# JuliaGenAI/ColBERT.jl

Hardware: AMD Instinct MI355X
Metric: queries/sec, top-1000 on 1M-passage corpus (higher is better)
Workload: dtype f32

## Files before the change

### colbert.jl_amd/csrc/search_kernels.hpp

```cpp
#pragma once
#include <hip/hip_fp16.h>

#include "common.hpp"

namespace clb {

typedef float f32x16 __attribute__((ext_vector_type(16)));
typedef float f32x4 __attribute__((ext_vector_type(4)));

constexpr int kDim = 128;
constexpr int kCentTileStride = 132;
constexpr int kMaxTopK = 16384;

static __global__ __launch_bounds__(128) void centroid_scores_kernel(const float* __restrict__ C,
                                                               const float* __restrict__ Q,
                                                               float* __restrict__ cells, int K, int T,
                                                               int TT, int n_tiles) {
    extern __shared__ __attribute__((aligned(16))) float lds[];
    const int wave = threadIdx.x >> 6, lane = threadIdx.x & 63;
    const int i = lane & 31, h = lane >> 5;
    const int b = blockIdx.y / TT, tt = blockIdx.y % TT;
    const int Tpad = TT * 32;
    float* my = lds + wave * (32 * kCentTileStride);

// ... 358 lines not shown
    uint32_t* bm = bitmap + (size_t)b * W;
    const int w0 = slice * (SB * 1024);
#pragma unroll
    for (int j = 0; j < SB; ++j) {
        const int wi = j * 1024 + tid;
        const uint32_t word = lbm[wi];
        if (w0 + wi < W) bm[w0 + wi] = word;
        int c = __popc(word);
#pragma unroll
        for (int o = 32; o > 0; o >>= 1) c += __shfl_xor(c, o, 64);
        if ((tid & 63) == 0 && c) atomicAdd(&cnt[j], c);
    }
    __syncthreads();
    if (tid < SB && slice * SB + tid < nblk)
        blocksum[(size_t)b * nblk + slice * SB + tid] = cnt[tid];
}

static __global__ __launch_bounds__(kScanBlock) void bitmap_count_kernel(const uint32_t* __restrict__ bitmap,
                                                                  int* __restrict__ blocksum, int W) {
    __shared__ int sh[8];
    const int b = blockIdx.y;
    const uint32_t* bm = bitmap + (size_t)b * W;
    const int w0 = (blockIdx.x * kScanBlock + threadIdx.x) * kWordsPerThread;
    int cnt = 0;
#pragma unroll
    for (int j = 0; j < kWordsPerThread; ++j)
        if (w0 + j < W) cnt += __popc(bm[w0 + j]);
    int total;
    (void)block_exclusive_scan_256(cnt, sh, total);
    if (threadIdx.x == 0) blocksum[(size_t)b * gridDim.x + blockIdx.x] = total;
}

static __global__ __launch_bounds__(kScanBlock) void bitmap_emit_kernel(uint32_t* __restrict__ bitmap,
                                                                 const int* __restrict__ blockcnt,
                                                                 uint32_t* __restrict__ cand,
                                                                 const uint32_t* __restrict__ doc_off,
                                                                 uint2* __restrict__ cand_hdr, int W,
                                                                 size_t cand_cap, int* __restrict__ ncand) {
    __shared__ int sh[8];
    const int b = blockIdx.y;
    int before = 0;
    {
        const int* bc = blockcnt + (size_t)b * gridDim.x;
        const int upto = blockIdx.x == 0 ? (int)gridDim.x : (int)blockIdx.x;
        int part = 0;
        for (int i = threadIdx.x; i < upto; i += kScanBlock) part += bc[i];
        int total_;
        (void)block_exclusive_scan_256(part, sh, total_);
        if (blockIdx.x == 0) { if (threadIdx.x == 0) ncand[b] = total_; }
        else before = total_;
    }
    uint32_t* bm = bitmap + (size_t)b * W;
    const int w0 = (blockIdx.x * kScanBlock + threadIdx.x) * kWordsPerThread;
    uint32_t w[kWordsPerThread];
    int cnt = 0;
#pragma unroll
    for (int j = 0; j < kWordsPerThread; ++j) {
        w[j] = (w0 + j < W) ? bm[w0 + j] : 0u;
        cnt += __popc(w[j]);
    }
    int total;
    int pos = block_exclusive_scan_256(cnt, sh, total) + before;
    uint32_t* out = cand + (size_t)b * cand_cap;
    uint2* hdr = cand_hdr + (size_t)b * cand_cap;
#pragma unroll
    for (int j = 0; j < kWordsPerThread; ++j) {
        uint32_t x = w[j];
        if (x) bm[w0 + j] = 0u;
        while (x) {
            const int bit = __ffs((int)x) - 1;
            x &= x - 1;
            if ((size_t)pos < cand_cap) {
                const uint32_t pid = (uint32_t)((w0 + j) * 32 + bit);
                out[pos] = pid;
                const uint32_t o = doc_off[pid];
                hdr[pos] = make_uint2(o, doc_off[pid + 1] - o);
            }
            ++pos;
        }
    }
}

template <int NBITS>
__device__ __forceinline__ float bucket_weight(uint32_t idx, const float (&w)[4], float wlane) {
    if constexpr (NBITS == 1) {
        return idx ? w[1] : w[0];
    } else if constexpr (NBITS == 2) {
        const float lo = (idx & 1) ? w[1] : w[0];
        const float hi = (idx & 1) ? w[3] : w[2];
        return (idx & 2) ? hi : lo;
    } else {
        return __shfl(wlane, (int)idx, 64);
    }
}

template <int NBITS>
__device__ __forceinline__ void decompress_lane_dims(const float* __restrict__ cent_row ,
                                                     const uint32_t (&R)[NBITS * 4], int g,
                                                     const float (&w)[4], float wlane, float (&x)[32]) {
    float p = 0.f;
#pragma unroll
    for (int s = 0; s < 32; ++s) {
        const int bitpos = 4 * s * NBITS;
        const uint32_t idx = (R[bitpos >> 5] >> ((bitpos & 31) + g * NBITS)) & ((1u << NBITS) - 1u);
        const float v = cent_row[4 * s] + bucket_weight<NBITS>(idx, w, wlane);
        x[s] = v;
        const float sq = v * v;
        p = p + sq;
    }
    const float a = p + __shfl_xor(p, 16, 64);
    const float n2 = a + __shfl_xor(a, 32, 64);
    const float den = sqrtf(n2) + FLT_EPSILON;
#pragma unroll
    for (int s = 0; s < 32; ++s) x[s] = x[s] / den;
}

__device__ __forceinline__ float div_by_reciprocal(float x, float den, float y) {
    const float q0 = x * y;
    const float r = fmaf(-den, q0, x);
    return fmaf(r, y, q0);
}

template <int NBITS>
constexpr int weight_table_floats() { return (1 << NBITS) * 32; }
template <int NBITS>
__device__ __forceinline__ void fill_weight_table(float* tbl, const float* __restrict__ weights) {
    for (int i = threadIdx.x; i < weight_table_floats<NBITS>(); i += blockDim.x) tbl[i] = weights[i >> 5];
}

template <int NBITS>
__device__ __forceinline__ void decompress_lane_dims_fast(const float* __restrict__ cent_row ,
                                                          const uint32_t (&R)[NBITS * 4], int g,
                                                          const float* __restrict__ tbl, float (&x)[32],
                                                          const float* ctile = nullptr, int r = 0) {
    float p = 0.f;
    const float* tbl_lane = tbl + (threadIdx.x & 31);
#pragma unroll
    for (int s = 0; s < 32; ++s) {
        const int bit0 = 4 * s * NBITS;
        const uint32_t idx = __builtin_amdgcn_ubfe(R[bit0 >> 5], (uint32_t)((bit0 & 31) + g * NBITS), (uint32_t)NBITS);
        const float c = ctile ? ctile[(s * 16 + (r ^ (s & 15))) * 4 + ((g + 2 * (((r >> 3) ^ ((s & 15) >> 3)) & 1)) & 3)] : cent_row[4 * s];
        const float val = c + tbl_lane[idx * 32];
        x[s] = val;
        const float sq = val * val;
        p = p + sq;
    }
    const float a = p + __shfl_xor(p, 16, 64);
    const float n2 = a + __shfl_xor(a, 32, 64);
    const float den = sqrtf(n2) + FLT_EPSILON;
    if (__builtin_expect(den > 1e-18f && den < 1e18f, 1)) {
        const float y = 1.0f / den;
#pragma unroll
        for (int s = 0; s < 32; ++s) x[s] = div_by_reciprocal(x[s], den, y);
    } else {
#pragma unroll
        for (int s = 0; s < 32; ++s) x[s] = x[s] / den;
    }
}

constexpr int kMaxMaskedRows = 256;

template <int NBITS>
static __global__ __launch_bounds__(256, 3) void score_exact_kernel(
    const float* __restrict__ C, const float* __restrict__ weights, const uint32_t* __restrict__ codes0,
    const uint8_t* __restrict__ residuals, const uint2* __restrict__ cand_hdr, const float* __restrict__ Q,
    const int* __restrict__ ncand, float* __restrict__ scores, int T, size_t cand_cap,
    const int* __restrict__ list , const int* __restrict__ nlist) {
    constexpr int RD = NBITS * 4;
    __shared__ float tbl[weight_table_floats<NBITS>()];
    __shared__ __attribute__((aligned(16))) float qlds[16 * 64 * 4];
    __shared__ __attribute__((aligned(16))) float ctiles[4 * 512 * 4];
    fill_weight_table<NBITS>(tbl, weights);
    const int b = blockIdx.y;
    const int lane = threadIdx.x & 63;
    const int r = lane & 15, g = lane >> 4;
    const int wave = threadIdx.x >> 6;
    const int wave_global = blockIdx.x * 4 + wave;
    const int nwaves = gridDim.x * 4;
    const int n = list ? nlist[b] : ncand[b];
    const int TT = (T + 31) >> 5;
    const uint2* hdr = cand_hdr + (size_t)b * cand_cap;
    const int* lst = list ? list + (size_t)b * cand_cap : nullptr;
    float* ctile = ctiles + wave * 2048;
    const int c4 = lane & 31, rhalf = lane >> 5;

    auto stage_q = [&](int tt) {
        for (int i = threadIdx.x; i < 16 * 64; i += 256) {
            const int k = i >> 6, l = i & 63;
            const int rr = l & 15, gg = l >> 4;
            const int t0 = tt * 32 + rr, t1 = t0 + 16;
            const float* qa = Q + ((size_t)b * T + (t0 < T ? t0 : T - 1)) * kDim + gg;
            const float* qb = Q + ((size_t)b * T + (t1 < T ? t1 : T - 1)) * kDim + gg;
            float4 v;
            v.x = t0 < T ? qa[8 * k] : 0.f;
            v.y = t1 < T ? qb[8 * k] : 0.f;
            v.z = t0 < T ? qa[8 * k + 4] : 0.f;
            v.w = t1 < T ? qb[8 * k + 4] : 0.f;
            *reinterpret_cast<float4*>(qlds + (size_t)i * 4) = v;
        }
    };
    const float4* qv = reinterpret_cast<const float4*>(qlds) + lane;

#define CLB_REP8(X) X(0) X(1) X(2) X(3) X(4) X(5) X(6) X(7)
#define CLB_ROW_DECL(m) float4 row##m;
#define CLB_ROW_LOAD(m)                                                                                        \
    {                                                                                                          \
        const uint32_t ca = __builtin_amdgcn_readlane(code_rows, 2 * m), cb = __builtin_amdgcn_readlane(code_rows, 2 * m + 1); \
        row##m = *reinterpret_cast<const float4*>(C + (size_t)(rhalf ? cb : ca) * kDim + 4 * c4);              \
    }
#define CLB_ROW_STORE(m)                                                                                       \
    {      \
        float* sl_ = ctile + (c4 * 16 + ((2 * m + rhalf) ^ (c4 & 15))) * 4;                                    \
        const int ro_ = 2 * ((((2 * m + rhalf) >> 3) ^ (c4 >> 3)) & 1);                                        \
        *reinterpret_cast<float2*>(sl_ + ro_) = make_float2(row##m.x, row##m.y);                               \
        *reinterpret_cast<float2*>(sl_ + (ro_ ^ 2)) = make_float2(row##m.z, row##m.w);                         \
    }

    for (int tt = 0; tt < TT; ++tt) {
        __syncthreads();
        stage_q(tt);
        __syncthreads();
        int slot_cur = wave_global < n ? (lst ? lst[wave_global] : wave_global) : 0;
        int slot_nxt = wave_global + nwaves < n ? (lst ? lst[wave_global + nwaves] : wave_global + nwaves) : 0;
        uint2 h_cur = hdr[slot_cur];
        for (int j = wave_global; j < n; j += nwaves) {
            const int slot = slot_cur;
            const uint32_t off = __builtin_amdgcn_readfirstlane(h_cur.x);
            const int len = (int)__builtin_amdgcn_readfirstlane(h_cur.y);
            {
                const int j1 = j + nwaves, j2 = j + 2 * nwaves;
                slot_cur = slot_nxt;
                if (j1 < n) h_cur = hdr[slot_nxt];
                slot_nxt = j2 < n ? (lst ? lst[j2] : j2) : 0;
            }
            float m0 = kNegInf, m1 = kNegInf;
            auto row_at = [&](int el) -> uint32_t { return (uint32_t)(el < len ? el : len - 1); };
            auto code_at = [&](int base) { return codes0[off + row_at(base + r)]; };
            uint32_t Rn[RD];
            auto load_res = [&](int base) {
                const uint32_t e = off + row_at(base + r);
                const uint32_t* rp = reinterpret_cast<const uint32_t*>(residuals + (size_t)e * (RD * 4));
#pragma unroll
                for (int k4 = 0; k4 < RD; k4 += 4) {
                    uint4 v = *reinterpret_cast<const uint4*>(rp + k4);
                    Rn[k4] = v.x; Rn[k4 + 1] = v.y; Rn[k4 + 2] = v.z; Rn[k4 + 3] = v.w;
                }
            };
            uint32_t code_rows = code_at(0);
            uint32_t code_next = code_at(16);
            load_res(0);
            CLB_REP8(CLB_ROW_DECL)
            CLB_REP8(CLB_ROW_LOAD)
            for (int base = 0; base < len; base += 16) {
                uint32_t R[RD];
#pragma unroll
                for (int k4 = 0; k4 < RD; ++k4) R[k4] = Rn[k4];
                CLB_REP8(CLB_ROW_STORE)
                __builtin_amdgcn_wave_barrier();
                if (base + 16 < len) load_res(base + 16);
                float x[32];
                decompress_lane_dims_fast<NBITS>(nullptr, R, g, tbl, x, ctile, r);
                __builtin_amdgcn_wave_barrier();
                code_rows = code_next;
                if (base + 16 < len) { CLB_REP8(CLB_ROW_LOAD) }
                code_next = code_at(base + 32);
                f32x4 a0 = {0.f, 0.f, 0.f, 0.f}, a1 = {0.f, 0.f, 0.f, 0.f};
                float4 qnext = qv[0];
#pragma unroll
                for (int k = 0; k < 16; ++k) {
                    const float4 q = qnext;
                    if (k < 15) qnext = qv[(k + 1) * 64];
                    a0 = __builtin_amdgcn_mfma_f32_16x16x4f32(x[2 * k], q.x, a0, 0, 0, 0);
                    a1 = __builtin_amdgcn_mfma_f32_16x16x4f32(x[2 * k], q.y, a1, 0, 0, 0);
                    a0 = __builtin_amdgcn_mfma_f32_16x16x4f32(x[2 * k + 1], q.z, a0, 0, 0, 0);
                    a1 = __builtin_amdgcn_mfma_f32_16x16x4f32(x[2 * k + 1], q.w, a1, 0, 0, 0);
                }
                m0 = fmaxf(fmaxf(m0, fmaxf(a0[0], a0[1])), fmaxf(a0[2], a0[3]));
                m1 = fmaxf(fmaxf(m1, fmaxf(a1[0], a1[1])), fmaxf(a1[2], a1[3]));
            }
            m0 = fmaxf(m0, __shfl_xor(m0, 16, 64));
            m0 = fmaxf(m0, __shfl_xor(m0, 32, 64));
            m1 = fmaxf(m1, __shfl_xor(m1, 16, 64));
            m1 = fmaxf(m1, __shfl_xor(m1, 32, 64));
            float total = tt == 0 ? 0.f : scores[(size_t)b * cand_cap + slot];
#pragma unroll
            for (int t = 0; t < 32; ++t) {
                const float v = __shfl(t < 16 ? m0 : m1, t & 15, 64);
                if (tt * 32 + t < T) total = total + v;
            }
            if (lane == 0) scores[(size_t)b * cand_cap + slot] = total;
        }
    }
#undef CLB_REP8
#undef CLB_ROW_DECL
#undef CLB_ROW_LOAD
#undef CLB_ROW_STORE
}

struct ExactStepTag {
    int slot;
    int slot1;
    int info;
};
__device__ __forceinline__ uint32_t nth_set_bit_256(unsigned long long w0, unsigned long long w1,
                                                    unsigned long long w2, unsigned long long w3, int n) {
    const int c0 = __popcll(w0), c1 = c0 + __popcll(w1), c2 = c1 + __popcll(w2);
    unsigned long long w = w0;
    int add = 0, loc = n;
    if (n >= c0) { w = w1; add = 64; loc = n - c0; }
    if (n >= c1) { w = w2; add = 128; loc = n - c1; }
    if (n >= c2) { w = w3; add = 192; loc = n - c2; }
    uint32_t x = (uint32_t)w;
    const int cl = __popc(x);
    if (loc >= cl) { x = (uint32_t)(w >> 32); add += 32; loc -= cl; }
#pragma unroll
    for (int width = 16; width >= 1; width >>= 1) {
        const int t = __popc(x & ((1u << width) - 1u));
        if (loc >= t) { x >>= width; add += width; loc -= t; }
    }
    return (uint32_t)add;
}

static __global__ __launch_bounds__(256, 3) void score_exact_flat_kernel(
    const float* __restrict__ C, const float* __restrict__ weights, const uint32_t* __restrict__ codes0,
    const uint8_t* __restrict__ residuals, const uint2* __restrict__ cand_hdr, const float* __restrict__ Q,
    float* __restrict__ scores, int T, size_t cand_cap, const int* __restrict__ list,
    const int* __restrict__ nlist, const unsigned long long* __restrict__ rowmask) {
    constexpr int NBITS = 2;
    __shared__ float tbl[weight_table_floats<NBITS>()];
    __shared__ __attribute__((aligned(16))) float qlds[16 * 64 * 4];
    __shared__ __attribute__((aligned(16))) float ctiles[4 * 512 * 4];
    fill_weight_table<NBITS>(tbl, weights);
    const int lane = threadIdx.x & 63;
    const int r = lane & 15, g = lane >> 4;
    const int wave = __builtin_amdgcn_readfirstlane(threadIdx.x >> 6);
    float* ctile = ctiles + wave * 2048;
    const int c4 = lane & 31, rhalf = lane >> 5;
    const float4* qv = reinterpret_cast<const float4*>(qlds) + lane;

#define CLB_REP8(X) X(0) X(1) X(2) X(3) X(4) X(5) X(6) X(7)
#define CLB_ROW_DECL(m) float4 rowA##m;
#define CLB_ROW_LOAD(P, CODE, m)                                                                               \
    {                                                                                                          \
        const uint32_t ca = __builtin_amdgcn_readlane(CODE, 2 * m), cb = __builtin_amdgcn_readlane(CODE, 2 * m + 1); \
        row##P##m = *reinterpret_cast<const float4*>(C + (size_t)(rhalf ? cb : ca) * kDim + 4 * c4);           \
    }
#define CLB_ROW_LOAD8(P, CODE)                                                                                 \
    CLB_ROW_LOAD(P, CODE, 0) CLB_ROW_LOAD(P, CODE, 1) CLB_ROW_LOAD(P, CODE, 2) CLB_ROW_LOAD(P, CODE, 3)        \
    CLB_ROW_LOAD(P, CODE, 4) CLB_ROW_LOAD(P, CODE, 5) CLB_ROW_LOAD(P, CODE, 6) CLB_ROW_LOAD(P, CODE, 7)
#define CLB_ROW_STORE(P, m)                                                                                    \
    {      \
        float* sl_ = ctile + (c4 * 16 + ((2 * m + rhalf) ^ (c4 & 15))) * 4;                                    \
        const int ro_ = 2 * ((((2 * m + rhalf) >> 3) ^ (c4 >> 3)) & 1);                                        \
        *reinterpret_cast<float2*>(sl_ + ro_) = make_float2(row##P##m.x, row##P##m.y);                         \
        *reinterpret_cast<float2*>(sl_ + (ro_ ^ 2)) = make_float2(row##P##m.z, row##P##m.w);                   \
    }
#define CLB_ROW_STORE8(P)                                                                                      \
    CLB_ROW_STORE(P, 0) CLB_ROW_STORE(P, 1) CLB_ROW_STORE(P, 2) CLB_ROW_STORE(P, 3)                            \
    CLB_ROW_STORE(P, 4) CLB_ROW_STORE(P, 5) CLB_ROW_STORE(P, 6) CLB_ROW_STORE(P, 7)

    {
        const int b = blockIdx.y;
        __syncthreads();
        for (int i = threadIdx.x; i < 16 * 64; i += 256) {
            const int k = i >> 6, l = i & 63;
            const int rr = l & 15, gg = l >> 4;
            const int t0 = rr, t1 = rr + 16;
            const float* qa = Q + ((size_t)b * T + (t0 < T ? t0 : T - 1)) * kDim + gg;
            const float* qb = Q + ((size_t)b * T + (t1 < T ? t1 : T - 1)) * kDim + gg;
            float4 v;
            v.x = t0 < T ? qa[8 * k] : 0.f;
            v.y = t1 < T ? qb[8 * k] : 0.f;
            v.z = t0 < T ? qa[8 * k + 4] : 0.f;
            v.w = t1 < T ? qb[8 * k + 4] : 0.f;
            *reinterpret_cast<float4*>(qlds + (size_t)i * 4) = v;
        }
        __syncthreads();
        const int n = nlist[b];
        const int* lst = list + (size_t)b * cand_cap;
        const uint2* hdr = cand_hdr + (size_t)b * cand_cap;
        const unsigned long long* mw = rowmask + (size_t)b * cand_cap * 4;
        float* out = scores + (size_t)b * cand_cap;
        const int stride = gridDim.x * 4;

        for (int j0 = blockIdx.x * 4 + wave; j0 < n; j0 += 64 * stride) {
            const int jl = j0 + lane * stride;
            const int jj = jl < n ? jl : j0;
            const int slot_l = lst[jj];
            const uint2 hv = hdr[slot_l];
            const unsigned long long mk0 = mw[(size_t)jj * 4], mk1 = mw[(size_t)jj * 4 + 1],
                                     mk2 = mw[(size_t)jj * 4 + 2], mk3 = mw[(size_t)jj * 4 + 3];
            const bool ident_l = (int)hv.y > kMaxMaskedRows;
            const uint32_t nj_l = ident_l ? (hv.y | 0x80000000u)
                                          : (uint32_t)(__popcll(mk0) + __popcll(mk1) + __popcll(mk2) + __popcll(mk3));
            const int nd = (n - j0 + stride - 1) / stride < 64 ? (n - j0 + stride - 1) / stride : 64;
            int it_k = 0, it_base = 0;
            uint32_t it_off, it_nj;
            int it_slot;
            unsigned long long it_m0, it_m1, it_m2, it_m3;
#define CLB_IT_LOAD(KK)                                                                                        \
    {                                                                                                          \
        it_off = __builtin_amdgcn_readlane(hv.x, KK);                                                          \
        it_nj = __builtin_amdgcn_readlane(nj_l, KK);                                                           \
        it_slot = __builtin_amdgcn_readlane(slot_l, KK);                                                       \
        it_m0 = ((unsigned long long)(uint32_t)__builtin_amdgcn_readlane((uint32_t)(mk0 >> 32), KK) << 32) | (uint32_t)__builtin_amdgcn_readlane((uint32_t)mk0, KK); \
        it_m1 = ((unsigned long long)(uint32_t)__builtin_amdgcn_readlane((uint32_t)(mk1 >> 32), KK) << 32) | (uint32_t)__builtin_amdgcn_readlane((uint32_t)mk1, KK); \
        it_m2 = ((unsigned long long)(uint32_t)__builtin_amdgcn_readlane((uint32_t)(mk2 >> 32), KK) << 32) | (uint32_t)__builtin_amdgcn_readlane((uint32_t)mk2, KK); \
        it_m3 = ((unsigned long long)(uint32_t)__builtin_amdgcn_readlane((uint32_t)(mk3 >> 32), KK) << 32) | (uint32_t)__builtin_amdgcn_readlane((uint32_t)mk3, KK); \
    }
            CLB_IT_LOAD(0)

#define CLB_XSTAGE_A(CODE, R0, R1, TAG)                                                                        \
    {                                                                                                          \
        const bool live = it_k < nd;                                                                           \
        const int nj = (int)(it_nj & 0x7fffffffu);                                                             \
        const int rem = nj - it_base;                                                                          \
        uint32_t e;                                                                                            \
        if (rem < 16 && it_k + 1 < nd) {                  \
            const int kn = it_k + 1;                                                                           \
            const uint32_t nx_off = __builtin_amdgcn_readlane(hv.x, kn);                                       \
            const uint32_t nx_nj = __builtin_amdgcn_readlane(nj_l, kn);                                        \
            const int nx_slot = __builtin_amdgcn_readlane(slot_l, kn);                                         \
            const unsigned long long nx_m0 = ((unsigned long long)(uint32_t)__builtin_amdgcn_readlane((uint32_t)(mk0 >> 32), kn) << 32) | (uint32_t)__builtin_amdgcn_readlane((uint32_t)mk0, kn); \
            const unsigned long long nx_m1 = ((unsigned long long)(uint32_t)__builtin_amdgcn_readlane((uint32_t)(mk1 >> 32), kn) << 32) | (uint32_t)__builtin_amdgcn_readlane((uint32_t)mk1, kn); \
            const unsigned long long nx_m2 = ((unsigned long long)(uint32_t)__builtin_amdgcn_readlane((uint32_t)(mk2 >> 32), kn) << 32) | (uint32_t)__builtin_amdgcn_readlane((uint32_t)mk2, kn); \
            const unsigned long long nx_m3 = ((unsigned long long)(uint32_t)__builtin_amdgcn_readlane((uint32_t)(mk3 >> 32), kn) << 32) | (uint32_t)__builtin_amdgcn_readlane((uint32_t)mk3, kn); \
            const int njn = (int)(nx_nj & 0x7fffffffu);                                                        \
            const int take = 16 - rem < njn ? 16 - rem : njn;                                                  \
            const bool second = r >= rem;                  \
            const int ia = it_base + r;                                                                        \
            const int ib = r - rem < njn ? r - rem : njn - 1;                                                  \
            const int idx = second ? ib : ia;                                                                  \
            const bool ident = ((second ? nx_nj : it_nj) & 0x80000000u) != 0u;                                 \
            const uint32_t row = ident ? (uint32_t)idx                                                         \
                                       : nth_set_bit_256(second ? nx_m0 : it_m0, second ? nx_m1 : it_m1,       \
                                                         second ? nx_m2 : it_m2, second ? nx_m3 : it_m3, idx); \
            e = (second ? nx_off : it_off) + row;                                                              \
            const int last1 = njn <= 16 - rem;                                                                 \
            TAG.slot = it_slot;                                                                                \
            TAG.slot1 = nx_slot;                                                                               \
            TAG.info = rem | 0x100 | (last1 << 9);                                                             \
            it_k += 1;                                                                                         \
            if (last1) {                                                                                       \
                it_k += 1;                                                                                     \
                const int kk = it_k < 64 ? it_k : 63;                                                          \
                CLB_IT_LOAD(kk)                                                                                \
                it_base = 0;                                                                                   \
            } else {                                                                                           \
                it_off = nx_off; it_nj = nx_nj; it_slot = nx_slot;                                             \
                it_m0 = nx_m0; it_m1 = nx_m1; it_m2 = nx_m2; it_m3 = nx_m3;                                    \
                it_base = take;                                                                                \
            }                                                                                                  \
        } else {                                                                                               \
            const int idx = it_base + r < nj ? it_base + r : nj - 1;                                           \
            const uint32_t row = (it_nj & 0x80000000u) ? (uint32_t)idx : nth_set_bit_256(it_m0, it_m1, it_m2, it_m3, idx); \
            e = live ? it_off + row : 0u;                                                                      \
            const int last = it_base + 16 >= nj;                                                               \
            TAG.slot = live ? it_slot : -1;                                                                    \
            TAG.slot1 = -1;                                                                                    \
            TAG.info = 16 | (last << 8);                                                                       \
            it_base += 16;                                                                                     \
            if (last) {                                                                                        \
                it_k += 1;                                                                                     \
                const int kk = it_k < 64 ? it_k : 63;                                                          \
                CLB_IT_LOAD(kk)                                                                                \
                it_base = 0;                                                                                   \
            }                                                                                                  \
        }                                                                                                      \
        CODE = codes0[e];                                                                                      \
        const uint4* rp = reinterpret_cast<const uint4*>(residuals + (size_t)e * 32);                          \
        R0 = rp[0];                                                                                            \
        R1 = rp[1];                                                                                            \
    }
#define CLB_XSTAGE_C(P, R0, R1, TAG, CODE_NEXT2)                                                               \
    {                                                                                                          \
        CLB_ROW_STORE8(P)                                                                                      \
        __builtin_amdgcn_wave_barrier();                                                                       \
        const uint32_t R[8] = {R0.x, R0.y, R0.z, R0.w, R1.x, R1.y, R1.z, R1.w};                                \
        float x[32];                                                                                           \
        decompress_lane_dims_fast<NBITS>(nullptr, R, g, tbl, x, ctile, r);                                     \
        __builtin_amdgcn_wave_barrier();                                                                       \
        CLB_ROW_LOAD8(P, CODE_NEXT2)                                                                           \
        f32x4 a0 = {0.f, 0.f, 0.f, 0.f}, a1 = {0.f, 0.f, 0.f, 0.f};                                            \
        float4 qnext = qv[0];                                                                                  \
        _Pragma("unroll") for (int k = 0; k < 16; ++k) {                                                       \
            const float4 q = qnext;                                                                            \
            if (k < 15) qnext = qv[(k + 1) * 64];                                                              \
            a0 = __builtin_amdgcn_mfma_f32_16x16x4f32(x[2 * k], q.x, a0, 0, 0, 0);                             \
            a1 = __builtin_amdgcn_mfma_f32_16x16x4f32(x[2 * k], q.y, a1, 0, 0, 0);                             \
            a0 = __builtin_amdgcn_mfma_f32_16x16x4f32(x[2 * k + 1], q.z, a0, 0, 0, 0);                         \
            a1 = __builtin_amdgcn_mfma_f32_16x16x4f32(x[2 * k + 1], q.w, a1, 0, 0, 0);                         \
        }                                                                                                      \
         \
         \
        float c0, c1, n0 = kNegInf, n1 = kNegInf;                                                              \
        const int p_ = TAG.info & 31;                                                                          \
        if (p_ >= 16) {                                                                                        \
            c0 = fmaxf(fmaxf(m0, fmaxf(a0[0], a0[1])), fmaxf(a0[2], a0[3]));                                   \
            c1 = fmaxf(fmaxf(m1, fmaxf(a1[0], a1[1])), fmaxf(a1[2], a1[3]));                                   \
        } else {                                                                                               \
            c0 = m0;                                                                                           \
            c1 = m1;                                                                                           \
            _Pragma("unroll") for (int q_ = 0; q_ < 4; ++q_) {                                                 \
                const bool first_ = 4 * g + q_ < p_;                                                           \
                c0 = fmaxf(c0, first_ ? a0[q_] : kNegInf);                                                     \
                c1 = fmaxf(c1, first_ ? a1[q_] : kNegInf);                                                     \
                n0 = fmaxf(n0, first_ ? kNegInf : a0[q_]);                                                     \
                n1 = fmaxf(n1, first_ ? kNegInf : a1[q_]);                                                     \
            }                                                                                                  \
        }                                                                                                      \
        {                                                                                                      \
            const int nfin_ = ((TAG.info >> 8) & 1) + ((TAG.info >> 9) & 1);        \
            int cs_ = TAG.slot;                                                                                \
            _Pragma("unroll 1") for (int f_ = 0; f_ < nfin_; ++f_) {                                           \
                c0 = fmaxf(c0, __shfl_xor(c0, 16, 64));                                                        \
                c0 = fmaxf(c0, __shfl_xor(c0, 32, 64));                                                        \
                c1 = fmaxf(c1, __shfl_xor(c1, 16, 64));                                                        \
                c1 = fmaxf(c1, __shfl_xor(c1, 32, 64));                                                        \
                 \
                 \
                 \
                float total = 0.f;                                                                             \
                _Pragma("unroll") for (int t = 0; t < 32; ++t) {                                               \
                    const uint32_t sv = __builtin_amdgcn_readlane(__float_as_uint(t < 16 ? c0 : c1), t & 15);  \
                    total = total + __uint_as_float(t < T ? sv : 0u);                                          \
                }                                                                                              \
                if (lane == 0 && cs_ >= 0) out[cs_] = total;                                                   \
                c0 = n0;                                                                                       \
                c1 = n1;                                                                                       \
                n0 = kNegInf;                                                                                  \
                n1 = kNegInf;                                                                                  \
                cs_ = TAG.slot1;                                                                               \
            }                                                                                                  \
        }                                                                                                      \
        m0 = c0;                                                                                               \
        m1 = c1;                                                                                               \
    }

            float m0 = kNegInf, m1 = kNegInf;
            uint32_t cd0, cd1, cd2;
            uint4 ra0, rb0, ra1, rb1, ra2, rb2;
            ExactStepTag t0, t1, t2;
            CLB_REP8(CLB_ROW_DECL)
            CLB_XSTAGE_A(cd0, ra0, rb0, t0)
            CLB_XSTAGE_A(cd1, ra1, rb1, t1)
            CLB_ROW_LOAD8(A, cd0)
            while (t0.slot >= 0) {
                CLB_XSTAGE_A(cd2, ra2, rb2, t2)
                CLB_XSTAGE_C(A, ra0, rb0, t0, cd1)
                CLB_XSTAGE_A(cd0, ra0, rb0, t0)
                CLB_XSTAGE_C(A, ra1, rb1, t1, cd2)
                CLB_XSTAGE_A(cd1, ra1, rb1, t1)
                CLB_XSTAGE_C(A, ra2, rb2, t2, cd0)
            }
#undef CLB_IT_LOAD
#undef CLB_XSTAGE_A
#undef CLB_XSTAGE_C
        }
    }
#undef CLB_REP8
#undef CLB_ROW_DECL
#undef CLB_ROW_LOAD
#undef CLB_ROW_LOAD8
#undef CLB_ROW_STORE
#undef CLB_ROW_STORE8
}

__device__ __forceinline__ void radix_pick(const int* hist, int rem, uint32_t prefix, int shift,
                                           uint32_t* s_prefix, int* s_remaining) {
    const int lane = threadIdx.x & 63;
    const int4 h = *reinterpret_cast<const int4*>(hist + 4 * lane);
    const int own = h.x + h.y + h.z + h.w;
    int x = own;
#pragma unroll
    for (int o = 1; o < 64; o <<= 1) {
        const int y = __shfl_down(x, o, 64);
        if (lane + o < 64) x += y;
    }
    int above = x - own;
    const int hv[4] = {h.x, h.y, h.z, h.w};
#pragma unroll
    for (int j = 3; j >= 0; --j) {
        if (above < rem && rem <= above + hv[j]) {
            *s_prefix = prefix | ((uint32_t)(4 * lane + j) << shift);
            *s_remaining = rem - above;
        }
        above += hv[j];
    }
}

constexpr int kSelCache = 32;

__device__ __forceinline__ void hist_add_aggregated(int* hist, uint32_t bin, bool active) {
    const int lane = threadIdx.x & 63;
    unsigned long long todo = __builtin_amdgcn_ballot_w64(active);
#pragma unroll 1
    for (int it = 0; it < 4 && todo != 0; ++it) {
        const int leader = __builtin_amdgcn_readfirstlane(__ffsll((long long)todo) - 1);
        const uint32_t lb = __builtin_amdgcn_readlane(bin, leader);
        const unsigned long long same = __builtin_amdgcn_ballot_w64(active && bin == lb) & todo;
        if (__popcll(same) < 8) break;
        if (lane == leader) atomicAdd(&hist[lb], (int)__popcll(same));
        todo &= ~same;
    }
    if ((todo >> lane) & 1ull) atomicAdd(&hist[bin], 1);
}

#define CLB_RADIX_SELECT() CLB_RADIX_SELECT_N(99)
#define CLB_RADIX_SELECT_N(LIMIT)                                                                           \
    {                                                                                                       \
        uint32_t kmin_ = 0xffffffffu, kmax_ = 0u;                                                           \
        CLB_SEL_FOR_EACH(if (valid) { kmin_ = key < kmin_ ? key : kmin_; kmax_ = key > kmax_ ? key : kmax_; }) \
        _Pragma("unroll") for (int o_ = 32; o_ > 0; o_ >>= 1) {                                             \
            const uint32_t a_ = __shfl_xor(kmin_, o_, 64), b_ = __shfl_xor(kmax_, o_, 64);                  \
            kmin_ = a_ < kmin_ ? a_ : kmin_;                                                                \
            kmax_ = b_ > kmax_ ? b_ : kmax_;                                                                \
        }                                                                                                   \
        if (tid == 0) { s_kmin = 0xffffffffu; s_kmax = 0u; }                                                \
        __syncthreads();                                                                                    \
        if ((tid & 63) == 0) { atomicMin(&s_kmin, kmin_); atomicMax(&s_kmax, kmax_); }                      \
        __syncthreads();                                                                                    \
        const uint32_t diff_ = s_kmin ^ s_kmax;                                                             \
        if (diff_ == 0u) {                                                                                  \
            if (tid == 0) s_prefix = s_kmax;                            \
            __syncthreads();                                                                                \
        } else {                                                                                            \
            const int top_ = 31 - __clz((int)diff_);                                                        \
            int shift_ = top_ > 7 ? top_ - 7 : 0;                                                           \
            int width_ = top_ - shift_ + 1;                                                                 \
            if (tid == 0) s_prefix = top_ == 31 ? 0u : (s_kmax & (0xffffffffu << (top_ + 1)));              \
            int passes_ = 0;                                                                                \
            for (;;) {                                                                                      \
                if (tid < 256) hist[tid] = 0;                                                               \
                __syncthreads();                                                                            \
                const uint32_t prefix_ = s_prefix;                                                          \
                const uint32_t himask_ = shift_ + width_ >= 32 ? 0u : (0xffffffffu << (shift_ + width_));   \
                const uint32_t bmask_ = (1u << width_) - 1u;                                                \
                CLB_SEL_FOR_EACH(hist_add_aggregated(hist, (key >> shift_) & bmask_,                        \
                                                     valid && (key & himask_) == prefix_);)                 \
                __syncthreads();                                                                            \
                if (tid < 64) radix_pick(hist, s_remaining, prefix_, shift_, &s_prefix, &s_remaining);      \
                __syncthreads();                                                                            \
                if (shift_ == 0 || ++passes_ >= (LIMIT)) break;                                             \
                const int ns_ = shift_ > 8 ? shift_ - 8 : 0;                                                \
                width_ = shift_ - ns_;                                                                      \
                shift_ = ns_;                                                                               \
            }                                                                                               \
        }                                                                                                   \
    }

constexpr int kRankMax = 4096;
constexpr int kRankBlocks = 8;

static __global__ __launch_bounds__(1024) void topk_kernel(const float* __restrict__ scores,
                                                    const uint32_t* __restrict__ cand,
                                                    const int* __restrict__ ncand,
                                                    const int* __restrict__ list,
                                                    const int* __restrict__ nlist, int k, int kpow2,
                                                    size_t cand_cap, int64_t pid_offset,
                                                    int64_t* __restrict__ out_pids,
                                                    float* __restrict__ out_scores,
                                                    int* __restrict__ short_flag,
                                                    int64_t* __restrict__ n_cand_out ,
                                                    int ranked_elsewhere = 0) {
    extern __shared__ __attribute__((aligned(16))) unsigned long long skeys[];
    __shared__ __attribute__((aligned(16))) int hist[256];
    __shared__ int sh_scan[32];
    __shared__ uint32_t s_prefix, s_kmin, s_kmax;
    __shared__ int s_remaining;
    const int b = blockIdx.x, tid = threadIdx.x;
    const int n = list ? nlist[b] : ncand[b];
    if (ranked_elsewhere && list && n <= kRankMax) return;
    const float* sc = scores + (size_t)b * cand_cap;
    const int* lst = list ? list + (size_t)b * cand_cap : nullptr;
    const int keff = n < k ? n : k;
    int kp = 1;
    while (kp < keff) kp <<= 1;
    kp = kp < kpow2 ? kp : kpow2;
    if (tid == 0) {
        short_flag[b] = n < k ? 1 : 0;
        if (n_cand_out) n_cand_out[b] = ncand[b];
    }

    const int chunk = (n + 1023) >> 10;
    const int i0 = tid * chunk;
    const bool cached = chunk <= kSelCache;
    uint32_t ckey[kSelCache];
    int cslot[kSelCache];
    if (cached) {
#pragma unroll
        for (int c = 0; c < kSelCache; ++c) {
            const int i = i0 + c;
            const bool valid = c < chunk && i < n;
            cslot[c] = valid ? (lst ? lst[i] : i) : 0;
            ckey[c] = valid ? f32_order_key(sc[cslot[c]]) : 0u;
        }
    }
#define CLB_SEL_FOR_EACH(...)                                                                   \
    if (cached) {                                                                               \
        _Pragma("unroll") for (int c = 0; c < kSelCache; ++c) {                                 \
            if (c >= chunk) break;                                                              \
            const bool valid = i0 + c < n;                                                      \
            const int slot = cslot[c];                                                          \
            const uint32_t key = ckey[c];                                                       \
            (void)slot;                                                                         \
            __VA_ARGS__                                                                         \
        }                                                                                       \
    } else {                                                                                    \
        for (int c = 0; c < chunk; ++c) {                                                       \
            const bool valid = i0 + c < n;                                                      \
            const int slot = valid ? (lst ? lst[i0 + c] : i0 + c) : 0;                          \
            const uint32_t key = valid ? f32_order_key(sc[slot]) : 0u;                          \
            (void)slot;                                                                         \
            __VA_ARGS__                                                                         \
        }                                                                                       \
    }

    if (tid == 0) { s_prefix = 0u; s_remaining = keff; }
    __syncthreads();
    if (keff > 0) {
        if (cached) {
            CLB_RADIX_SELECT()
        } else {
#pragma push_macro("CLB_SEL_FOR_EACH")
#undef CLB_SEL_FOR_EACH
#define CLB_SEL_FOR_EACH(...)                                                                   \
    for (int c = 0; c < chunk; ++c) {                                                           \
        const int i_ = c * 1024 + tid;                                                          \
        const bool valid = i_ < n;                                                              \
        const uint32_t key = valid ? f32_order_key(sc[lst ? lst[i_] : i_]) : 0u;                \
        __VA_ARGS__                                                                             \
    }
            CLB_RADIX_SELECT()
#pragma pop_macro("CLB_SEL_FOR_EACH")
        }
    }
    const uint32_t tau = s_prefix;
    const int need_eq = s_remaining;

    for (int i = tid; i < kp; i += 1024) skeys[i] = 0ull;
    __syncthreads();
    if (keff > 0) {
        int ngt = 0, neq = 0;
        CLB_SEL_FOR_EACH(ngt += valid && key > tau; neq += valid && key == tau;)
        const int lane = tid & 63, wave = tid >> 6;
        int xg = ngt, xe = neq;
#pragma unroll
        for (int o = 1; o < 64; o <<= 1) {
            const int yg = __shfl_up(xg, o, 64), ye = __shfl_up(xe, o, 64);
            if (lane >= o) { xg += yg; xe += ye; }
        }
        if (lane == 63) { sh_scan[wave] = xg; sh_scan[16 + wave] = xe; }
        __syncthreads();
        int gt_before = xg - ngt, eq_rank = xe - neq;
        for (int w2 = 0; w2 < wave; ++w2) { gt_before += sh_scan[w2]; eq_rank += sh_scan[16 + w2]; }
        CLB_SEL_FOR_EACH(
            if (valid) {
                const bool gt = key > tau, eq = key == tau;
                if (gt || (eq && eq_rank < need_eq)) {
                    const int pos = gt_before + (eq_rank < need_eq ? eq_rank : need_eq);
                    skeys[pos] = ((unsigned long long)key << 32) | (unsigned long long)(0xffffffffu - (uint32_t)slot);
                }
                gt_before += gt;
                eq_rank += eq;
            })
    }
#undef CLB_SEL_FOR_EACH
    __syncthreads();
    for (int size = 2; size <= kp; size <<= 1) {
        for (int stride = size >> 1; stride > 0; stride >>= 1) {
            if (stride >= 64 || (kp >> 1) > 1024) __syncthreads();
            else __builtin_amdgcn_wave_barrier();
            for (int i = tid; i < (kp >> 1); i += 1024) {
                const int lo = 2 * i - (i & (stride - 1));
                const int hi = lo + stride;
                const bool desc = (lo & size) == 0;
                const unsigned long long a = skeys[lo], c = skeys[hi];
                if ((a < c) == desc) { skeys[lo] = c; skeys[hi] = a; }
            }
        }
    }
    __syncthreads();
    const uint32_t* cnd = cand + (size_t)b * cand_cap;
    for (int i = tid; i < k; i += 1024) {
        int64_t pid = 0;
        float s = kNegInf;
        if (i < keff) {
            const unsigned long long key = skeys[i];
            const uint32_t slot = 0xffffffffu - (uint32_t)(key & 0xffffffffull);
            pid = pid_offset + (int64_t)cnd[slot] + 1;
            s = sc[slot];
        }
        out_pids[(size_t)b * k + i] = pid;
        out_scores[(size_t)b * k + i] = s;
    }
}

static __global__ __launch_bounds__(1024) void topk_rank_kernel(const float* __restrict__ scores,
                                                                const uint32_t* __restrict__ cand,
                                                                const int* __restrict__ ncand,
                                                                const int* __restrict__ list,
                                                                const int* __restrict__ nlist, int k, size_t cand_cap,
                                                                int64_t pid_offset, int64_t* __restrict__ out_pids,
                                                                float* __restrict__ out_scores,
                                                                int* __restrict__ short_flag,
                                                                int64_t* __restrict__ n_cand_out ) {
    __shared__ __attribute__((aligned(16))) unsigned long long keys[kRankMax];
    __shared__ int ranks[256];
    const int b = blockIdx.y, g = blockIdx.x, tid = threadIdx.x;
    const int n = nlist[b];
    if (n > kRankMax) return;
    const float* sc = scores + (size_t)b * cand_cap;
    const int* lst = list + (size_t)b * cand_cap;
    const int keff = n < k ? n : k;
    if (g == 0) {
        if (tid == 0) {
            short_flag[b] = n < k ? 1 : 0;
            if (n_cand_out) n_cand_out[b] = ncand[b];
        }
        for (int i = keff + tid; i < k; i += 1024) {
            out_pids[(size_t)b * k + i] = 0;
            out_scores[(size_t)b * k + i] = kNegInf;
        }
    }
    for (int i = tid; i < n; i += 1024) {
        const int slot = lst[i];
        keys[i] = ((unsigned long long)f32_order_key(sc[slot]) << 32) | (unsigned long long)(0xffffffffu - (uint32_t)slot);
    }
    __syncthreads();
    const uint32_t* cnd = cand + (size_t)b * cand_cap;
    const int e = tid & 255, quarter = __builtin_amdgcn_readfirstlane(tid >> 8);
    const int q0 = (int)(((long long)n * quarter) >> 2), q1 = (int)(((long long)n * (quarter + 1)) >> 2);
    for (int base = g * 256; base < n; base += kRankBlocks * 256) {
        const int i = base + e;
        if (tid < 256) ranks[tid] = 0;
        __syncthreads();
        const unsigned long long mine = i < n ? keys[i] : ~0ull;
        int cnt = 0;
#pragma unroll 4
        for (int j = q0; j < q1; ++j) cnt += keys[j] > mine;
        if (cnt) atomicAdd(&ranks[e], cnt);
        __syncthreads();
        if (tid < 256 && i < n) {
            const int r = ranks[e];
            if (r < keff) {
                const uint32_t slot = 0xffffffffu - (uint32_t)(mine & 0xffffffffull);
                out_pids[(size_t)b * k + r] = pid_offset + (int64_t)cnd[slot] + 1;
                out_scores[(size_t)b * k + r] = sc[slot];
            }
        }
        __syncthreads();
    }
}

static __global__ void ivf_to_pid_kernel(const int64_t* __restrict__ ivf, const uint32_t* __restrict__ doc_off,
                                  uint32_t* __restrict__ ivf_pid, int64_t n_emb, int n_docs,
                                  int* __restrict__ err) {
// ... 136 lines not shown
```

Measured before the change: 30760.

## Precompute per-wave LDS row lists instead of nth-set-bit search per lane

Replaces the per-lane nth_set_bit_256 popcount search over 256-bit row masks with a per-wave LDS byte list of active row indices, built once per batch of candidates using mbcnt prefix counts. The stage loop then looks up rows by prefix offset and no longer carries four 64-bit mask registers per candidate. Batches are now cut short when the list would overflow 1024 entries, so the outer loop advances by the number of candidates actually consumed. It also moves the T masking of the final sum out of the 32-step readlane loop. In exchange it adds a serial list-build loop, LDS usage and wave barriers.

```diff
diff --git a/colbert.jl_amd/csrc/search_kernels.hpp b/colbert.jl_amd/csrc/search_kernels.hpp
--- a/colbert.jl_amd/csrc/search_kernels.hpp
+++ b/colbert.jl_amd/csrc/search_kernels.hpp
@@ -684,24 +684,7 @@
     int slot1;
     int info;
 };
-__device__ __forceinline__ uint32_t nth_set_bit_256(unsigned long long w0, unsigned long long w1,
-                                                    unsigned long long w2, unsigned long long w3, int n) {
-    const int c0 = __popcll(w0), c1 = c0 + __popcll(w1), c2 = c1 + __popcll(w2);
-    unsigned long long w = w0;
-    int add = 0, loc = n;
-    if (n >= c0) { w = w1; add = 64; loc = n - c0; }
-    if (n >= c1) { w = w2; add = 128; loc = n - c1; }
-    if (n >= c2) { w = w3; add = 192; loc = n - c2; }
-    uint32_t x = (uint32_t)w;
-    const int cl = __popc(x);
-    if (loc >= cl) { x = (uint32_t)(w >> 32); add += 32; loc -= cl; }
-#pragma unroll
-    for (int width = 16; width >= 1; width >>= 1) {
-        const int t = __popc(x & ((1u << width) - 1u));
-        if (loc >= t) { x >>= width; add += width; loc -= t; }
-    }
-    return (uint32_t)add;
-}
+constexpr int kRowList = 1024;
 
 static __global__ __launch_bounds__(256, 3) void score_exact_flat_kernel(
     const float* __restrict__ C, const float* __restrict__ weights, const uint32_t* __restrict__ codes0,
@@ -712,11 +695,13 @@
     __shared__ float tbl[weight_table_floats<NBITS>()];
     __shared__ __attribute__((aligned(16))) float qlds[16 * 64 * 4];
     __shared__ __attribute__((aligned(16))) float ctiles[4 * 512 * 4];
+    __shared__ uint8_t rowlists[4 * kRowList];
     fill_weight_table<NBITS>(tbl, weights);
     const int lane = threadIdx.x & 63;
     const int r = lane & 15, g = lane >> 4;
     const int wave = __builtin_amdgcn_readfirstlane(threadIdx.x >> 6);
     float* ctile = ctiles + wave * 2048;
+    uint8_t* rl = rowlists + wave * kRowList;
     const int c4 = lane & 31, rhalf = lane >> 5;
     const float4* qv = reinterpret_cast<const float4*>(qlds) + lane;
 
@@ -765,7 +750,7 @@
         float* out = scores + (size_t)b * cand_cap;
         const int stride = gridDim.x * 4;
 
-        for (int j0 = blockIdx.x * 4 + wave; j0 < n; j0 += 64 * stride) {
+        for (int j0 = blockIdx.x * 4 + wave; j0 < n;) {
             const int jl = j0 + lane * stride;
             const int jj = jl < n ? jl : j0;
             const int slot_l = lst[jj];
@@ -775,20 +760,41 @@
             const bool ident_l = (int)hv.y > kMaxMaskedRows;
             const uint32_t nj_l = ident_l ? (hv.y | 0x80000000u)
                                           : (uint32_t)(__popcll(mk0) + __popcll(mk1) + __popcll(mk2) + __popcll(mk3));
-            const int nd = (n - j0 + stride - 1) / stride < 64 ? (n - j0 + stride - 1) / stride : 64;
+            const int nd_all = (n - j0 + stride - 1) / stride < 64 ? (n - j0 + stride - 1) / stride : 64;
+            __builtin_amdgcn_wave_barrier();
+            int pfx_l = 0, nd = 0, used = 0;
+            for (; nd < nd_all; ++nd) {
+                const uint32_t njk = __builtin_amdgcn_readlane(nj_l, nd);
+                const int ne = (njk & 0x80000000u) ? 0 : (njk != 0u ? (int)njk : 1);
+                if (used + ne > kRowList) break;
+                int pos = used + (njk == 0u ? 1 : 0);
+                pfx_l = lane == nd ? pos : pfx_l;
+                used += ne;
+                if (ne == 0) continue;
+                if (njk == 0u) {
+                    if (lane == 0) rl[pos - 1] = 0;
+                    continue;
+                }
+#define CLB_RL_WORD(W, Q)                                                                                      \
+    {                                                                                                          \
+        const uint32_t lo_ = __builtin_amdgcn_readlane((uint32_t)(W), nd), hi_ = __builtin_amdgcn_readlane((uint32_t)((W) >> 32), nd); \
+        const unsigned long long w_ = ((unsigned long long)hi_ << 32) | lo_;                                   \
+        if ((w_ >> lane) & 1ull) rl[pos + (int)__builtin_amdgcn_mbcnt_hi(hi_, __builtin_amdgcn_mbcnt_lo(lo_, 0u))] = (uint8_t)(64 * (Q) + lane); \
+        pos += __popcll(w_);                                                                                   \
+    }
+                CLB_RL_WORD(mk0, 0) CLB_RL_WORD(mk1, 1) CLB_RL_WORD(mk2, 2) CLB_RL_WORD(mk3, 3)
+#undef CLB_RL_WORD
+            }
+            __builtin_amdgcn_wave_barrier();
             int it_k = 0, it_base = 0;
             uint32_t it_off, it_nj;
-            int it_slot;
-            unsigned long long it_m0, it_m1, it_m2, it_m3;
+            int it_slot, it_pfx;
 #define CLB_IT_LOAD(KK)                                                                                        \
     {                                                                                                          \
         it_off = __builtin_amdgcn_readlane(hv.x, KK);                                                          \
         it_nj = __builtin_amdgcn_readlane(nj_l, KK);                                                           \
         it_slot = __builtin_amdgcn_readlane(slot_l, KK);                                                       \
-        it_m0 = ((unsigned long long)(uint32_t)__builtin_amdgcn_readlane((uint32_t)(mk0 >> 32), KK) << 32) | (uint32_t)__builtin_amdgcn_readlane((uint32_t)mk0, KK); \
-        it_m1 = ((unsigned long long)(uint32_t)__builtin_amdgcn_readlane((uint32_t)(mk1 >> 32), KK) << 32) | (uint32_t)__builtin_amdgcn_readlane((uint32_t)mk1, KK); \
-        it_m2 = ((unsigned long long)(uint32_t)__builtin_amdgcn_readlane((uint32_t)(mk2 >> 32), KK) << 32) | (uint32_t)__builtin_amdgcn_readlane((uint32_t)mk2, KK); \
-        it_m3 = ((unsigned long long)(uint32_t)__builtin_amdgcn_readlane((uint32_t)(mk3 >> 32), KK) << 32) | (uint32_t)__builtin_amdgcn_readlane((uint32_t)mk3, KK); \
+        it_pfx = __builtin_amdgcn_readlane(pfx_l, KK);                                                         \
     }
             CLB_IT_LOAD(0)
 
@@ -803,10 +809,7 @@
             const uint32_t nx_off = __builtin_amdgcn_readlane(hv.x, kn);                                       \
             const uint32_t nx_nj = __builtin_amdgcn_readlane(nj_l, kn);                                        \
             const int nx_slot = __builtin_amdgcn_readlane(slot_l, kn);                                         \
-            const unsigned long long nx_m0 = ((unsigned long long)(uint32_t)__builtin_amdgcn_readlane((uint32_t)(mk0 >> 32), kn) << 32) | (uint32_t)__builtin_amdgcn_readlane((uint32_t)mk0, kn); \
-            const unsigned long long nx_m1 = ((unsigned long long)(uint32_t)__builtin_amdgcn_readlane((uint32_t)(mk1 >> 32), kn) << 32) | (uint32_t)__builtin_amdgcn_readlane((uint32_t)mk1, kn); \
-            const unsigned long long nx_m2 = ((unsigned long long)(uint32_t)__builtin_amdgcn_readlane((uint32_t)(mk2 >> 32), kn) << 32) | (uint32_t)__builtin_amdgcn_readlane((uint32_t)mk2, kn); \
-            const unsigned long long nx_m3 = ((unsigned long long)(uint32_t)__builtin_amdgcn_readlane((uint32_t)(mk3 >> 32), kn) << 32) | (uint32_t)__builtin_amdgcn_readlane((uint32_t)mk3, kn); \
+            const int nx_pfx = __builtin_amdgcn_readlane(pfx_l, kn);                                           \
             const int njn = (int)(nx_nj & 0x7fffffffu);                                                        \
             const int take = 16 - rem < njn ? 16 - rem : njn;                                                  \
             const bool second = r >= rem;                  \
@@ -814,9 +817,8 @@
             const int ib = r - rem < njn ? r - rem : njn - 1;                                                  \
             const int idx = second ? ib : ia;                                                                  \
             const bool ident = ((second ? nx_nj : it_nj) & 0x80000000u) != 0u;                                 \
-            const uint32_t row = ident ? (uint32_t)idx                                                         \
-                                       : nth_set_bit_256(second ? nx_m0 : it_m0, second ? nx_m1 : it_m1,       \
-                                                         second ? nx_m2 : it_m2, second ? nx_m3 : it_m3, idx); \
+            const uint32_t lrow = rl[((second ? nx_pfx : it_pfx) + idx) & (kRowList - 1)];                     \
+            const uint32_t row = ident ? (uint32_t)idx : lrow;                                                 \
             e = (second ? nx_off : it_off) + row;                                                              \
             const int last1 = njn <= 16 - rem;                                                                 \
             TAG.slot = it_slot;                                                                                \
@@ -829,13 +831,12 @@
                 CLB_IT_LOAD(kk)                                                                                \
                 it_base = 0;                                                                                   \
             } else {                                                                                           \
-                it_off = nx_off; it_nj = nx_nj; it_slot = nx_slot;                                             \
-                it_m0 = nx_m0; it_m1 = nx_m1; it_m2 = nx_m2; it_m3 = nx_m3;                                    \
+                it_off = nx_off; it_nj = nx_nj; it_slot = nx_slot; it_pfx = nx_pfx;                            \
                 it_base = take;                                                                                \
             }                                                                                                  \
         } else {                                                                                               \
             const int idx = it_base + r < nj ? it_base + r : nj - 1;                                           \
-            const uint32_t row = (it_nj & 0x80000000u) ? (uint32_t)idx : nth_set_bit_256(it_m0, it_m1, it_m2, it_m3, idx); \
+            const uint32_t row = (it_nj & 0x80000000u) ? (uint32_t)idx : (uint32_t)rl[(it_pfx + idx) & (kRowList - 1)]; \
             e = live ? it_off + row : 0u;                                                                      \
             const int last = it_base + 16 >= nj;                                                               \
             TAG.slot = live ? it_slot : -1;                                                                    \
@@ -902,11 +903,11 @@
                  \
                  \
                  \
+                 \
+                const float s0_ = r < T ? c0 : 0.f, s1_ = r + 16 < T ? c1 : 0.f;                                  \
                 float total = 0.f;                                                                             \
-                _Pragma("unroll") for (int t = 0; t < 32; ++t) {                                               \
-                    const uint32_t sv = __builtin_amdgcn_readlane(__float_as_uint(t < 16 ? c0 : c1), t & 15);  \
-                    total = total + __uint_as_float(t < T ? sv : 0u);                                          \
-                }                                                                                              \
+                _Pragma("unroll") for (int t = 0; t < 32; ++t)                                                 \
+                    total = total + __uint_as_float(__builtin_amdgcn_readlane(__float_as_uint(t < 16 ? s0_ : s1_), t & 15)); \
                 if (lane == 0 && cs_ >= 0) out[cs_] = total;                                                   \
                 c0 = n0;                                                                                       \
                 c1 = n1;                                                                                       \
@@ -935,6 +936,7 @@
                 CLB_XSTAGE_A(cd1, ra1, rb1, t1)
                 CLB_XSTAGE_C(A, ra2, rb2, t2, cd0)
             }
+            j0 += nd * stride;
 #undef CLB_IT_LOAD
 #undef CLB_XSTAGE_A
 #undef CLB_XSTAGE_C
```

After: 31000, median of 6. About the same (+0.8%).
